# Audio-WestlakeU/NBSS

Hardware: AMD Instinct MI355X
Metric: utterances/sec (4 s, 6ch, 129 freqs) SpatialNet bf16 train at 1/2/4/8 MI355X (higher is better)
Workload: dtype bf16; 1 GPU; SpatialNet-small 6ch->2spk, 4-s 8-kHz utterances (32000 samples), n_fft 256/hop 128 (F=129, T=251), 8 layers, full train step (STFT..Adam), bf16 stream + fp32 master/stats, 32 utterances per GPU per step; batch_per_gpu=32, global_batch=32, parallelism=dp1

## Files before the change

nbss_amd/csrc/common.h:

```cpp
#pragma once
#ifdef NBSS_EMU
#include "hipemu.h"
#define NBSS_LDS(name) char* name = hipemu::g_block->lds
#else
#include <hip/hip_runtime.h>
#define NBSS_LDS(name) extern __shared__ __attribute__((aligned(16))) char name[]
#endif
#include <stdint.h>

typedef unsigned short bf16_t;
typedef float f32x4 __attribute__((ext_vector_type(4)));
typedef float f32x2 __attribute__((ext_vector_type(2)));
typedef short s16x8 __attribute__((ext_vector_type(8)));
typedef short s16x4 __attribute__((ext_vector_type(4)));
typedef unsigned int u32x2 __attribute__((ext_vector_type(2)));
typedef unsigned int u32x4 __attribute__((ext_vector_type(4)));

#define NBSS_DEV __device__ __forceinline__

NBSS_DEV float bf2f(bf16_t h) {
    union { uint32_t u; float f; } c;
    c.u = ((uint32_t)h) << 16;
    return c.f;
}
// ... 11 lines not shown
NBSS_DEV uint32_t pack2bf(float a, float b) {
    typedef __bf16 bf16x2_t __attribute__((ext_vector_type(2)));
    typedef float f32x2_t __attribute__((ext_vector_type(2)));
    f32x2_t v = {a, b};
    return __builtin_bit_cast(uint32_t, __builtin_convertvector(v, bf16x2_t));
}
#endif

NBSS_DEV float keep_if(bool c, float v) { return c ? v : 0.f; }

NBSS_DEV float fast_exp2(float x) {
#ifdef NBSS_EMU
    return exp2f(x);
#else
    return __builtin_amdgcn_exp2f(x);
#endif
}

NBSS_DEV float silu_f(float x) { return x / (1.0f + __expf(-x)); }
NBSS_DEV float dsilu_f(float x) {
    float s = 1.0f / (1.0f + __expf(-x));
    return s * (1.0f + x * (1.0f - s));
}

NBSS_DEV float fast_rcp(float x) {
#ifdef NBSS_EMU
    return 1.0f / x;
#else
    return __builtin_amdgcn_rcpf(x);
#endif
}
NBSS_DEV float sigmoid_fast(float x) { return fast_rcp(1.0f + fast_exp2(-1.44269504f * x)); }
NBSS_DEV float silu_fast(float x) { return x * sigmoid_fast(x); }
NBSS_DEV float dsilu_fast(float x) {
    const float s = sigmoid_fast(x);
    return s * (1.0f + x * (1.0f - s));
}
NBSS_DEV void silu_pair(float x, float& y, float& dy) {
    const float s = sigmoid_fast(x);
    y = x * s;
    dy = s * (1.0f + x * (1.0f - s));
}

NBSS_DEV void lds_barrier() {
#ifdef NBSS_EMU
    __syncthreads();
#else
    __builtin_amdgcn_s_waitcnt(0xC07F);
    __builtin_amdgcn_s_barrier();
#endif
}

NBSS_DEV float opaque(float x) {
#ifndef NBSS_EMU
    asm volatile("" : "+v"(x));
#endif
    return x;
}

NBSS_DEV void sched_fence() {
#ifndef NBSS_EMU
    __builtin_amdgcn_sched_barrier(0);
#endif
}

NBSS_DEV void wave_lds_sync() {
#ifdef NBSS_EMU
    hipemu::wave_sync();
#else
    __builtin_amdgcn_fence(__ATOMIC_RELEASE, "wavefront");
    __builtin_amdgcn_wave_barrier();
    __builtin_amdgcn_fence(__ATOMIC_ACQUIRE, "wavefront");
#endif
}

NBSS_DEV void dma16_to_lds(void* lds_wave_base, const void* g) {
#ifdef NBSS_EMU
    uint32_t* d = reinterpret_cast<uint32_t*>(reinterpret_cast<char*>(lds_wave_base) + 16 * (threadIdx.x & 63));
    const uint32_t* s = reinterpret_cast<const uint32_t*>(g);
    d[0] = s[0]; d[1] = s[1]; d[2] = s[2]; d[3] = s[3];
#else
    __builtin_amdgcn_global_load_lds((const __attribute__((address_space(1))) void*)g, (__attribute__((address_space(3))) void*)lds_wave_base, 16, 0, 0);
#endif
}
NBSS_DEV void dma_wait_all() {
#ifndef NBSS_EMU
    __builtin_amdgcn_s_waitcnt(0x0F70);
#endif
}

NBSS_DEV int lane_id() { return (int)(threadIdx.x & 63); }
NBSS_DEV int wave_id() { return (int)(threadIdx.x >> 6); }
NBSS_DEV int wave_id_u() {
#ifdef NBSS_EMU
    return (int)(threadIdx.x >> 6);
#else
    return __builtin_amdgcn_readfirstlane((int)(threadIdx.x >> 6));
#endif
}

NBSS_DEV float wave_sum16(float v) {
    v += __shfl_xor(v, 16);
    v += __shfl_xor(v, 32);
    return v;
}
NBSS_DEV float wave_max16(float v) {
// ... 220 lines not shown
```

nbss_amd/csrc/fconv.hip:

```cpp
#include "launch.h"
#include "layout.h"
#include "prof.h"
#include "blocks.h"
#include "wgrad.h"
#include "fold.h"
#include "foldk.h"
#include "geom.h"
#include "side.h"
#include <cstdlib>

#define FC_H 96
#define FC_G 8
#define FC_CG 12
#define FC_KS 2
#define FC_MTF_MAX 10
#define FC_MTF_BIG 17
#define FC_P16 (5 * FC_H * FC_CG)

template <class T> struct VecOf;
template <> struct VecOf<bf16_t> { static constexpr int N = 8; };
template <> struct VecOf<float> { static constexpr int N = 4; };

NBSS_DEV void vec_copy(bf16_t* d, const bf16_t* s) { *reinterpret_cast<u32x4*>(d) = *reinterpret_cast<const u32x4*>(s); }
NBSS_DEV void vec_copy(float* d, const float* s) { *reinterpret_cast<f32x4*>(d) = *reinterpret_cast<const f32x4*>(s); }
// ... 193 lines not shown

    if constexpr (REGX) {
#pragma unroll
        for (int k = 0; k < NXR; ++k) {
            const int i = tid + k * NTHR, f = i / VPR, off = (i % VPR) * VN, tt = off / HH;
            if (i >= F * VPR || t0 + tt >= T_) continue;
            const size_t go = (((size_t)b * F + f) * T_ + t0) * HH + off;
            float yv[8], o[8];
            load8(u + (size_t)f * ROW + tt * HHP + (off - tt * HH), yv);
#pragma unroll
            for (int j = 0; j < 4; ++j) {
                o[2 * j] = bf2f((bf16_t)(xr[k][j] & 0xFFFF)) + yv[2 * j];
                o[2 * j + 1] = bf2f((bf16_t)(xr[k][j] >> 16)) + yv[2 * j + 1];
            }
            store8(reinterpret_cast<bf16_t*>(y) + go, o);
        }
        for (int i = tid + NXR * NTHR; i < F * VPR; i += NTHR) {
            const int f = i / VPR, off = (i % VPR) * VN, tt = off / HH;
            if (t0 + tt >= T_) continue;
            const size_t go = (((size_t)b * F + f) * T_ + t0) * HH + off;
            float xv[8], yv[8], o[8];
            load8(x + go, xv);
            load8(u + (size_t)f * ROW + tt * HHP + (off - tt * HH), yv);
#pragma unroll
            for (int j = 0; j < 8; ++j) o[j] = xv[j] + yv[j];
            store8(reinterpret_cast<bf16_t*>(y) + go, o);
        }
    } else
    for (int i = tid; i < F * VPR; i += nthr) {
        const int f = i / VPR, off = (i % VPR) * VN, tt = off / HH;
        if (t0 + tt >= T_) continue;
        const size_t go = (((size_t)b * F + f) * T_ + t0) * HH + off;
        float xv[8], yv[8];
        if (VN == 8) {
            load8(x + go, xv);
            load8(u + (size_t)f * ROW + tt * HHP + (off - tt * HH), yv);
            float o[8];
#pragma unroll
            for (int j = 0; j < 8; ++j) o[j] = xv[j] + yv[j];
            store4(y + go, o[0], o[1], o[2], o[3]);
            store4(y + go + 4, o[4], o[5], o[6], o[7]);
        } else {
            load4(x + go, xv);
            load4(u + (size_t)f * ROW + tt * HHP + (off - tt * HH), yv);
            store4(y + go, xv[0] + yv[0], xv[1] + yv[1], xv[2] + yv[2], xv[3] + yv[3]);
        }
    }
}


#define FC_LD 104

template <class T>
NBSS_DEV void fconv_bfrag(Frag<T>& bq, const T* __restrict__ u, int rstride, int f, int ch0, int ks) {
    const int g4 = lane_id() >> 4;
    const int p0 = ks * 8 + 2 * g4, p1 = p0 + 1;
    frag_load_lo(bq, u + (size_t)(f + p0 / 3) * rstride + ch0 + (p0 % 3) * 4);
    if (p1 < 15) frag_load_hi(bq, u + (size_t)(f + p1 / 3) * rstride + ch0 + (p1 % 3) * 4);
    else frag_zero_hi(bq);
}

template <class T, bool WGF>
__global__ __launch_bounds__(64 * FC_G, 2)
void fconv_bwd_kernel(nbss_cfg c, const float* __restrict__ lnw, const float* __restrict__ lnb, const float* __restrict__ cb,
                      const float* __restrict__ slope, float* __restrict__ part, const T* __restrict__ Wp, const T* __restrict__ WpT,
                      const T* __restrict__ x, const T* __restrict__ dy, T* __restrict__ dx, float* __restrict__ stats, T* __restrict__ dvout, int flip) {
    constexpr int TT = 1, NW = FC_G;
    NBSS_LDS(smem);
    const int F = c.F, T_ = c.T, ntt = cdiv(T_, TT);
    const int bid = flip_bid(flip);
    const int b = bid / ntt, t0 = (bid % ntt) * TT;
    const int mtf = cdiv(F, 16), FP = mtf * 16 + 4, ntile = mtf * TT;
    constexpr int ROW = TT * FC_LD;
    T* u = reinterpret_cast<T*>(smem);
    T* dvb = u + (size_t)FP * ROW;
    float* aff = reinterpret_cast<float*>(dvb + (size_t)FP * ROW);
    float* lnp = aff + 3 * FC_H;
    float* affw = lnp + 2 * FC_H;
    PHASE_BEGIN(affw + NW * 2 * FC_H);
    const int tid = threadIdx.x, lane = lane_id(), l15 = lane & 15, g4 = lane >> 4, w = wave_id();
    constexpr bool DMA = sizeof(T) == 2;

    Frag<T> af[FC_KS], at[FC_KS];
#pragma unroll
    for (int ks = 0; ks < FC_KS; ++ks) {
        wfrag_load(af[ks], Wp, w < FC_G ? w : 0, FC_KS, ks);
        wfrag_load(at[ks], WpT, w < FC_G ? w : 0, FC_KS, ks);
    }
    for (int i = tid; i < 3 * FC_H; i += blockDim.x) aff[i] = 0.f;
    for (int i = tid; i < NW * 2 * FC_H; i += blockDim.x) affw[i] = 0.f;
    for (int i = tid; i < 2 * FC_H; i += blockDim.x) lnp[i] = i < FC_H ? lnw[i] : lnb[i - FC_H];
    constexpr int VZ = VecOf<T>::N;
    for (int i = tid; i < 4 * ROW / VZ; i += blockDim.x) {
        const int e = i * VZ, hr = e / ROW, rr = hr < 2 ? hr : mtf * 16 + hr, off = e % ROW;
        vec_zero(u + (size_t)rr * ROW + off);
        vec_zero(dvb + (size_t)rr * ROW + off);
    }

    auto row_load = [&](int ti, Frag<T> (&xq)[BK_KS], Frag<T> (&dq)[BK_KS]) {
        const int ft = ti / TT, tt = ti % TT, f = ft * 16 + l15, t = t0 + tt;
        const bool valid = f < F && t < T_;
        const size_t n = ((size_t)b * F + f) * T_ + t;
#pragma unroll
        for (int ks = 0; ks < BK_KS; ++ks) {
            if (valid) {
                frag_load(xq[ks], x + n * FC_H + ks * 32 + 8 * g4);
                frag_load(dq[ks], dy + n * FC_H + ks * 32 + 8 * g4);
            } else {
                frag_zero(xq[ks]);
                frag_zero(dq[ks]);
            }
        }
    };
    auto row_stats = [&](const Frag<T> (&xq)[BK_KS], float& mean, float& rstd) {
        float sum = 0.f;
#pragma unroll
        for (int ks = 0; ks < BK_KS; ++ks)
#pragma unroll
            for (int j = 0; j < 8; ++j) sum += frag_get(xq[ks], j);
        mean = wave_sum16(sum) * (1.0f / FC_H);
        float q = 0.f;
#pragma unroll
        for (int ks = 0; ks < BK_KS; ++ks)
#pragma unroll
            for (int j = 0; j < 8; ++j) {
                const float d = frag_get(xq[ks], j) - mean;
                q += d * d;
            }
        rstd = rsqrtf(wave_sum16(q) * (1.0f / FC_H) + 1e-5f);
    };
    auto row_fwd = [&](int ti, const Frag<T> (&xq)[BK_KS], const Frag<T> (&dq)[BK_KS], float mean, float rstd) {
        const int ft = ti / TT, tt = ti % TT, f = ft * 16 + l15, t = t0 + tt;
        const bool valid = f < F && t < T_;
        if (!WGF && valid && g4 == 0) {
            const size_t n = ((size_t)b * F + f) * T_ + t;
            stats[n * 2] = mean;
            stats[n * 2 + 1] = rstd;
        }
        T* ur = u + (size_t)(f + 2) * ROW + tt * FC_LD;
        T* dr_ = dvb + (size_t)(f + 2) * ROW + tt * FC_LD;
#pragma unroll
        for (int ks = 0; ks < BK_KS; ++ks) {
            const int c0 = ks * 32 + 8 * g4;
            float gm[8], bt[8], o[8], d[8];
            load8(lnp + c0, gm);
            load8(lnp + FC_H + c0, bt);
#pragma unroll
            for (int j = 0; j < 8; ++j) {
                o[j] = valid ? (frag_get(xq[ks], j) - mean) * rstd * gm[j] + bt[j] : 0.f;
                d[j] = frag_get(dq[ks], j);
            }
            store8(ur + c0, o);
            if (!DMA) store8(dr_ + c0, d);
        }
    };
    Frag<T> xr[BK_KS], dr[BK_KS];
    float rmean = 0.f, rrstd = 0.f;
    if constexpr (DMA) {
        const int wu = wave_id_u(), Q = F * TT * 13;
        for (int i = wu; i * 64 < Q; i += NW) {
            const int q = i * 64 + lane, r = q / 13, cc = q - r * 13, f = r / TT, tt = r - f * TT;
            if (q < Q && cc < 12 && t0 + tt < T_) {
                const size_t n = ((size_t)b * F + f) * T_ + t0 + tt;
                dma16_to_lds(reinterpret_cast<char*>(u + 2 * ROW) + (size_t)i * 1024, x + n * FC_H + cc * 8);
                dma16_to_lds(reinterpret_cast<char*>(dvb + 2 * ROW) + (size_t)i * 1024, dy + n * FC_H + cc * 8);
            }
        }
        for (int i = tid; i < (mtf * 16 - F) * ROW / VZ; i += blockDim.x) {
            vec_zero(u + (size_t)(F + 2) * ROW + i * VZ);
            vec_zero(dvb + (size_t)(F + 2) * ROW + i * VZ);
        }
        if (t0 + TT > T_)
            for (int i = tid; i < F * FC_LD / VZ; i += blockDim.x) {
                const int f = i / (FC_LD / VZ), e = (i % (FC_LD / VZ)) * VZ;
                for (int tt = T_ - t0; tt < TT; ++tt) {
                    vec_zero(u + (size_t)(f + 2) * ROW + tt * FC_LD + e);
                    vec_zero(dvb + (size_t)(f + 2) * ROW + tt * FC_LD + e);
                }
            }
        dma_wait_all();
        lds_barrier();
        auto row_load_lds = [&](int ti, Frag<T> (&xq)[BK_KS], Frag<T> (&dq)[BK_KS]) {
            const int ft = ti / TT, tt = ti % TT, f = ft * 16 + l15;
#pragma unroll
            for (int ks = 0; ks < BK_KS; ++ks) {
                frag_load(xq[ks], u + (size_t)(f + 2) * ROW + tt * FC_LD + ks * 32 + 8 * g4);
                frag_load(dq[ks], dvb + (size_t)(f + 2) * ROW + tt * FC_LD + ks * 32 + 8 * g4);
            }
        };
        if (w < ntile) {
            row_load_lds(w, xr, dr);
            row_stats(xr, rmean, rrstd);
            row_fwd(w, xr, dr, rmean, rrstd);
        }
        for (int ti = w + NW; ti < ntile; ti += NW) {
            Frag<T> xq[BK_KS], dq[BK_KS];
            float mean, rstd;
            row_load_lds(ti, xq, dq);
            row_stats(xq, mean, rstd);
            row_fwd(ti, xq, dq, mean, rstd);
        }
    } else {
    if (w < ntile) row_load(w, xr, dr);
    lds_barrier();
    if (w < ntile) {
        row_stats(xr, rmean, rrstd);
        row_fwd(w, xr, dr, rmean, rrstd);
    }
    for (int ti = w + NW; ti < ntile; ti += NW) {
        Frag<T> xq[BK_KS], dq[BK_KS];
        float mean, rstd;
        row_load(ti, xq, dq);
        row_stats(xq, mean, rstd);
        row_fwd(ti, xq, dq, mean, rstd);
    }
    }
    PHASE(0);
    lds_barrier();
    PHASE(1);

    const int ch = w * FC_CG + 4 * g4;
    const bool cvalid = g4 < 3;
    float cbv[4] = {0.f, 0.f, 0.f, 0.f}, slv[4] = {0.f, 0.f, 0.f, 0.f}, dsl[4] = {0.f, 0.f, 0.f, 0.f};
    if (cvalid) {
#pragma unroll
        for (int r = 0; r < 4; ++r) { cbv[r] = cb[ch + r]; slv[r] = slope[ch + r]; }
    }
    for (int ti = 0; ti < ntile; ++ti) {
        const int ft = ti / TT, tt = ti % TT, f = ft * 16 + l15;
        f32x4 acc = F32X4_ZERO;
#pragma unroll
        for (int ks = 0; ks < FC_KS; ++ks) {
            Frag<T> bq;
            fconv_bfrag<T>(bq, u + tt * FC_LD, ROW, f, w * FC_CG, ks);
            acc = mma(af[ks], bq, acc);
        }
        if (cvalid) {
            T* pd = dvb + (size_t)(f + 2) * ROW + tt * FC_LD + ch;
            float dyv[4], dv[4];
            load4(pd, dyv);
#pragma unroll
            for (int r = 0; r < 4; ++r) {
                const float v = acc[r] + cbv[r];
                dv[r] = v > 0.f ? dyv[r] : slv[r] * dyv[r];
                if (v <= 0.f) dsl[r] += dyv[r] * v;
            }
            store4(pd, dv[0], dv[1], dv[2], dv[3]);
        }
    }
#pragma unroll
    for (int r = 0; r < 4; ++r) {
        const float s2 = row_sum16(dsl[r]);
        if (l15 == 0 && cvalid) atomicAdd(aff + 2 * FC_H + ch + r, s2);
    }
    PHASE(2);
    lds_barrier();
    PHASE(3);

    constexpr int PROW = 4 * FC_H;
    if constexpr (WGF) {
        f32x4 wacc[5], bsum = F32X4_ZERO;
#pragma unroll
        for (int tap = 0; tap < 5; ++tap) wacc[tap] = F32X4_ZERO;
        Frag<T> ones;
#pragma unroll
        for (int jq = 0; jq < 8; ++jq) frag_set(ones, jq, 1.0f);
        const int nk = cdiv(mtf * 16, 32);
        const bool odd = (mtf & 1) != 0;
        const int roff = (4 * g4 + (l15 >> 2)) * ROW + w * FC_CG + 4 * (l15 & 3);
        for (int tt = 0; tt < TT; ++tt)
            for (int ks = 0; ks < nk; ++ks) {
                const bool half = odd && ks == nk - 1;
                Frag<T> fa;
                frag_load_tr(fa, dvb + (size_t)(2 + 32 * ks) * ROW + tt * FC_LD + roff, ROW);
                if (half) frag_zero_hi(fa);
                bsum = mma(fa, ones, bsum);
#pragma unroll
                for (int tap = 0; tap < 5; ++tap) {
                    Frag<T> fb;
                    frag_load_tr(fb, u + (size_t)(32 * ks + tap) * ROW + tt * FC_LD + roff, ROW);
                    if (half) frag_zero_hi(fb);
                    wacc[tap] = mma(fa, fb, wacc[tap]);
                }
            }
        bf16_t* prow16 = reinterpret_cast<bf16_t*>(part + (size_t)gridDim.x * PROW) + (size_t)bid * FC_P16;
        float* pb = part + (size_t)bid * PROW + 3 * FC_H;
        if (l15 < FC_CG && g4 < 3) {
#pragma unroll
            for (int tap = 0; tap < 5; ++tap) {
                const u32x2 v = {pack2bf(wacc[tap][0], wacc[tap][1]), pack2bf(wacc[tap][2], wacc[tap][3])};
                *reinterpret_cast<u32x2*>(prow16 + ((size_t)(tap * FC_G + w) * FC_CG + l15) * FC_CG + 4 * g4) = v;
            }
            if (l15 == 0) {
#pragma unroll
                for (int r = 0; r < 4; ++r) pb[w * FC_CG + 4 * g4 + r] = bsum[r];
            }
        }
    }

    for (int ti = 0; ti < ntile; ++ti) {
        const int ft = ti / TT, tt = ti % TT, f = ft * 16 + l15;
        f32x4 acc = F32X4_ZERO;
#pragma unroll
        for (int ks = 0; ks < FC_KS; ++ks) {
            Frag<T> bq;
            fconv_bfrag<T>(bq, dvb + tt * FC_LD, ROW, f, w * FC_CG, ks);
            acc = mma(at[ks], bq, acc);
        }
        if (cvalid) store4(u + (size_t)(f + 2) * ROW + tt * FC_LD + ch, acc[0], acc[1], acc[2], acc[3]);
    }
    if (!WGF) {
        constexpr int VN = VecOf<T>::N, VPR = FC_H / VN;
        for (int i = tid; i < F * TT * VPR; i += blockDim.x) {
            const int f = i / (TT * VPR), rem = i % (TT * VPR), tt = rem / VPR, off = (rem % VPR) * VN;
            if (t0 + tt < T_) vec_copy(dvout + (((size_t)b * F + f) * T_ + t0 + tt) * FC_H + off, dvb + (size_t)(f + 2) * ROW + tt * FC_LD + off);
        }
    }
    PHASE(4);
    lds_barrier();
    PHASE(5);

    auto row_bwd = [&](int ti, const Frag<T> (&xq)[BK_KS], const Frag<T> (&dq)[BK_KS], float mean, float rstd0) {
        const int ft = ti / TT, tt = ti % TT, f = ft * 16 + l15, t = t0 + tt;
        const bool valid = f < F && t < T_;
        const size_t n = ((size_t)b * F + f) * T_ + t;
        const T* ur = u + (size_t)(f + 2) * ROW + tt * FC_LD;
        const float rstd = valid ? rstd0 : 0.f;
        float m1 = 0.f, m2 = 0.f;
        static_assert(BK_KS == 3, "three k-steps of 32 channels");
        float* aw = affw + w * 2 * FC_H;
        float va[16];
        auto ks_vals = [&](int ks, float (&dvv)[8], float (&xhv)[8], bool stats) {
            const int c0 = ks * 32 + 8 * g4;
            float duv[8], gm[8];
            load8(ur + c0, duv);
            if (stats) load8(lnp + c0, gm);
#pragma unroll
            for (int j = 0; j < 8; ++j) {
                dvv[j] = valid ? duv[j] : 0.f;
                xhv[j] = (frag_get(xq[ks], j) - mean) * rstd;
                if (stats) {
                    m1 += dvv[j] * gm[j];
                    m2 += dvv[j] * gm[j] * xhv[j];
                }
            }
        };
        {
            float dvv[8], xhv[8];
#pragma unroll
            for (int ks = 0; ks < 2; ++ks) {
                ks_vals(ks, dvv, xhv, true);
#pragma unroll
                for (int j = 0; j < 8; ++j) va[8 * ks + j] = dvv[j] * xhv[j];
            }
            const float r0 = row_reduce16x16(va);
            aw[(l15 >> 3) * 32 + 8 * g4 + (l15 & 7)] += r0;
            ks_vals(2, dvv, xhv, true);
#pragma unroll
            for (int j = 0; j < 8; ++j) va[j] = dvv[j] * xhv[j];
#pragma unroll
            for (int j = 0; j < 8; ++j) va[8 + j] = dvv[j];
            const float r1 = row_reduce16x16(va);
            aw[(l15 >> 3) * FC_H + 64 + 8 * g4 + (l15 & 7)] += r1;
#pragma unroll
            for (int ks = 0; ks < 2; ++ks) {
                ks_vals(ks, dvv, xhv, false);
#pragma unroll
                for (int j = 0; j < 8; ++j) va[8 * ks + j] = dvv[j];
            }
            const float r2 = row_reduce16x16(va);
            aw[FC_H + (l15 >> 3) * 32 + 8 * g4 + (l15 & 7)] += r2;
        }
        m1 = wave_sum16(m1) * (1.0f / FC_H);
        m2 = wave_sum16(m2) * (1.0f / FC_H);
        if (valid) {
#pragma unroll
            for (int ks = 0; ks < BK_KS; ++ks) {
                const int c0 = ks * 32 + 8 * g4;
                float duv[8], gm[8], o[8];
                load8(ur + c0, duv);
                load8(lnp + c0, gm);
#pragma unroll
                for (int j = 0; j < 8; ++j) {
                    const float xh = (frag_get(xq[ks], j) - mean) * rstd;
                    o[j] = frag_get(dq[ks], j) + rstd * (duv[j] * gm[j] - m1 - xh * m2);
                }
                store8(dx + n * FC_H + c0, o);
            }
        }
    };
    if (w < ntile) row_bwd(w, xr, dr, rmean, rrstd);
    for (int ti = w + NW; ti < ntile; ti += NW) {
        Frag<T> xq[BK_KS], dq[BK_KS];
        float mean, rstd;
        row_load(ti, xq, dq);
        row_stats(xq, mean, rstd);
        row_bwd(ti, xq, dq, mean, rstd);
    }
    PHASE(6);
    lds_barrier();
    for (int i = threadIdx.x; i < 3 * FC_H; i += blockDim.x) {
        float v = aff[i];
        if (i < 2 * FC_H)
            for (int k = 0; k < NW; ++k) v += affw[k * 2 * FC_H + i];
        part[(size_t)bid * (WGF ? PROW : 3 * FC_H) + i] = v;
    }
    PHASE(7);
    PHASE_END();
}
PHASE_READER(nbss_phase_read_fconv_bwd)

template <class T, bool WGF>
static int fconv_bwd_t(const nbss_cfg& c, const float* P, float* part, const void* packed, int layer, int which, const void* x, const void* dy, void* dx,
                       float* stats, void* dv, hipStream_t st) {
    const int mtf = cdiv(c.F, 16);
    if (mtf > FC_MTF_BIG) return NBSS_EUNSUPPORTED;
    const size_t lds = (size_t)2 * (mtf * 16 + 4) * FC_LD * sizeof(T) + (5 + 2 * FC_G) * FC_H * sizeof(float) + PHASE_LDS_BYTES;
    if (lds > 160 * 1024) return NBSS_EUNSUPPORTED;
    const int lw = which ? P_FC2_LN_W : P_FC1_LN_W, lb = which ? P_FC2_LN_B : P_FC1_LN_B, sl = which ? P_FC2_PRELU : P_FC1_PRELU;
    const T* pk = (const T*)packed;
    int e = NBSS_SET_MAX_LDS((fconv_bwd_kernel<T, WGF>), lds);
    if (e) return e;
    dim3 grid(c.B * c.T), block(64 * FC_G);
    ProfScope ps(PK_FCONV_B, st);
    NBSS_LAUNCH((fconv_bwd_kernel<T, WGF>), grid, block, lds, st, c, P + param_off(c, layer, lw), P + param_off(c, layer, lb),
                P + param_off(c, layer, which ? P_FC2_B : P_FC1_B), P + param_off(c, layer, sl), part, pk + pack_off(c, layer, which ? K_FC2 : K_FC1),
                pk + pack_off(c, layer, which ? K_FC2_T : K_FC1_T), (const T*)x, (const T*)dy, (T*)dx, stats, (T*)dv, walk_flip_next());
    return NBSS_CHECK_LAUNCH();
}


#define TV_RSL_MAX 64
int part16_slices_launch(const void* part16, int nrows, float* slices, int p16, int* nsl, hipStream_t st, bool batch);
static_assert(FC_H == FK_H && FC_CG == FK_FCG && FC_G == FK_FG && FC_P16 == FK_FC_P16, "foldk.h");
__global__ __launch_bounds__(256) void fconv_part_final_kernel(const float* __restrict__ slices, int nsl, float* __restrict__ dW) {
    fk_fconv_final(slices, nsl, dW, (int)blockIdx.x);
}

int fconv_bwd_impl(const nbss_cfg& c, const float* P, float* G, const void* packed, int layer, int which, const void* x, const void* dy, void* dx,
                   void* ws, hipStream_t st, const Side* sd) {
    if (c.H != FC_H) return gb_fconv_bwd(c, P, G, layer, which, x, dy, dx, ws, st, sd);
    const size_t N = (size_t)c.B * c.F * c.T;
    float* stats = (float*)ws;
    void* dv = (char*)ws + ws_align(N * 2 * sizeof(float));
    float* part = (float*)((char*)ws + ws_part_offset(c));
    const bool big = c.F > 16 * FC_MTF_MAX;
    const bool fused = c.dtype == NBSS_BF16 && !big;
    if (fused) part = (float*)((char*)ws + ws_fcpart_offset(c));
    int e = c.dtype != NBSS_BF16 ? fconv_bwd_t<float, false>(c, P, part, packed, layer, which, x, dy, dx, stats, dv, st)
            : fused              ? fconv_bwd_t<bf16_t, true>(c, P, part, packed, layer, which, x, dy, dx, stats, dv, st)
                                 : fconv_bwd_t<bf16_t, false>(c, P, part, packed, layer, which, x, dy, dx, stats, dv, st);
    if (e) return e;
    const int nwg = c.B * c.T;
    AffSegs sg;
    sg.off[0] = param_off(c, layer, which ? P_FC2_LN_W : P_FC1_LN_W); sg.cnt[0] = FC_H;
    sg.off[1] = param_off(c, layer, which ? P_FC2_LN_B : P_FC1_LN_B); sg.cnt[1] = FC_H;
    sg.off[2] = param_off(c, layer, which ? P_FC2_PRELU : P_FC1_PRELU); sg.cnt[2] = FC_H;
    sg.n = fused ? 4 : 3;
    sg.off[3] = param_off(c, layer, which ? P_FC2_B : P_FC1_B); sg.cnt[3] = FC_H;
    const hipStream_t gs = side_fork(sd, st);
    FoldScope fs(gs, (char*)ws + ws_wgpart_offset(c), WGPART_BYTES, N);
    if ((e = affine_reduce_launch(part, nwg, sg, G, gs))) return e;
    if (fused) {
        float* slices = (float*)((char*)ws + ws_wgpart_offset(c));
        bool batch = false;
        if (g_fold) {
            int err;
            void* sl = g_fold->alloc((size_t)TV_RSL_MAX * FC_P16 * sizeof(float), &err);
            if (err) return err;
            if (sl) {
                slices = (float*)sl;
                batch = true;
            } else if ((err = g_fold->flush())) {
                return err;
            }
        }
        int nsl = 0;
        if ((e = part16_slices_launch(part + (size_t)nwg * 4 * FC_H, nwg, slices, FC_P16, &nsl, gs, batch))) return e;
        if (batch) {
            FoldItem it;
            it.kind = FK_FCONV_FINAL;
            it.gx = (FC_P16 + 255) / 256; it.gy = 1; it.nblk = it.gx;
            it.u.p16.part16 = nullptr; it.u.p16.nrows = nwg; it.u.p16.p16 = FC_P16; it.u.p16.nsl = nsl; it.u.p16.slices = slices;
            it.u.p16.G = G + param_off(c, layer, which ? P_FC2_W : P_FC1_W);
            if ((e = g_fold->add(2, it))) return e;
            return fs.end();
        }
        NBSS_FOLD_LAUNCH(fconv_part_final_kernel, dim3((FC_P16 + 255) / 256), dim3(256), 0, gs, (const float*)slices, nsl, G + param_off(c, layer, which ? P_FC2_W : P_FC1_W));
        return NBSS_CHECK_LAUNCH();
    }
    WgradArgs a;
    a.part = (float*)((char*)ws + ws_wgpart_offset(c));
    a.mvalid = 0; a.nvalid = 0;
    a.Ntok = (int)N; a.F = c.F; a.T = c.T; a.shift_stride = c.T; a.shift_dim = 1; a.groups = c.f_groups; a.taps = c.f_ks;
    a.A = dv; a.lda = FC_H; a.MA = FC_H; a.B = x; a.ldb = FC_H; a.NB = FC_H;
    a.stats = stats; a.gamma = P + param_off(c, layer, which ? P_FC2_LN_W : P_FC1_LN_W); a.beta = P + param_off(c, layer, which ? P_FC2_LN_B : P_FC1_LN_B);
    a.dW = G + param_off(c, layer, which ? P_FC2_W : P_FC1_W); a.dbias = G + param_off(c, layer, which ? P_FC2_B : P_FC1_B);
    if ((e = wgrad_launch(a, c.dtype, gs))) return e;
    return fs.end();
}

template <class T, int TT, int GPW, int MTF, int HH>
static int fconv_fwd_t(const nbss_cfg& c, const float* P, const void* packed, int layer, int which, const void* x, void* y, hipStream_t st) {
    const int mtf = cdiv(c.F, 16);
    if (mtf > MTF) return NBSS_EUNSUPPORTED;
    const size_t lds = (size_t)(mtf * 16 + 4) * TT * (HH + 8) * sizeof(T);
    if (lds > 160 * 1024) return NBSS_EUNSUPPORTED;
    const float* lnw = P + param_off(c, layer, which ? P_FC2_LN_W : P_FC1_LN_W);
    const float* lnb = P + param_off(c, layer, which ? P_FC2_LN_B : P_FC1_LN_B);
    const float* cb = P + param_off(c, layer, which ? P_FC2_B : P_FC1_B);
    const float* sl = P + param_off(c, layer, which ? P_FC2_PRELU : P_FC1_PRELU);
    const T* Wp = (const T*)packed + pack_off(c, layer, which ? K_FC2 : K_FC1);
    int e = NBSS_SET_MAX_LDS((fconv_fwd_kernel<T, TT, GPW, MTF, HH>), lds);
    if (e) return e;
    dim3 grid(c.B * cdiv(c.T, TT)), block(64 * FC_G / GPW);
// ... 20 lines not shown
```

nbss_amd/csrc/layout.h:

```cpp
#pragma once
#include "../../include/nbss_hip.h"

#ifdef NBSS_EMU
#define NBSS_HD inline
#else
#define NBSS_HD __host__ __device__ inline
#endif

enum LayerParam {
    P_FC1_LN_W, P_FC1_LN_B, P_FC1_W, P_FC1_B, P_FC1_PRELU,
    P_FULL_LN_W, P_FULL_LN_B, P_SQ_W, P_SQ_B, P_FULL_W, P_FULL_B, P_USQ_W, P_USQ_B,
    P_FC2_LN_W, P_FC2_LN_B, P_FC2_W, P_FC2_B, P_FC2_PRELU,
    P_MH_LN_W, P_MH_LN_B, P_INP_W, P_INP_B, P_OUTP_W, P_OUTP_B,
    P_TF_LN_W, P_TF_LN_B, P_TF_W1, P_TF_B1, P_TF_C1W, P_TF_C1B, P_TF_C2W, P_TF_C2B,
    P_TF_GN_W, P_TF_GN_B, P_TF_C3W, P_TF_C3B, P_TF_W2, P_TF_B2,
    NUM_LAYER_PARAMS
};

NBSS_HD int64_t layer_param_numel(const nbss_cfg& c, int p) {
    const int64_t H = c.H, FFN = c.FFN, SQ = c.SQ, F = c.F;
    switch (p) {
        case P_FC1_LN_W: case P_FC1_LN_B: case P_FC2_LN_W: case P_FC2_LN_B:
        case P_FULL_LN_W: case P_FULL_LN_B: case P_MH_LN_W: case P_MH_LN_B:
        case P_TF_LN_W: case P_TF_LN_B:
// ... 119 lines not shown
        case K_TF_W1_T: g.MT = c.H / 16; g.KS = c.t_groups * cdiv(cg, 32); break;
        case K_TF_C1_T: case K_TF_C2_T: case K_TF_C3_T: g.MT = cdiv(cg, 32) * 2; g.KS = cdiv(c.t_ks * (cg / 4), 8); g.NB = c.t_groups; break;
        case K_TF_W2_T: g.MT = c.t_groups * cdiv(cg, 32) * 2; g.KS = c.H / 32; break;
        case K_TF_W1_TN: g.MT = c.H / 16; g.KS = c.FFN / 32; break;
        case K_INP_TN: g.MT = c.H / 16; g.KS = 3 * c.H / 32; break;
        case K_TS_W1: g.MT = 1; g.KS = c.H / 16 + 1; g.NB = c.t_groups; break;
        case K_TS_W2_T: g.MT = 1; g.KS = c.H / 16; g.NB = c.t_groups; break;
        case K_TS_C1: case K_TS_C2: case K_TS_C3: case K_TS_C1_T: case K_TS_C2_T: case K_TS_C3_T:
            g.MT = 1; g.KS = cdiv(c.t_ks * (cg / 8) + 1, 2); g.NB = c.t_groups; break;
        case K_TS_W2: g.MT = c.H / 32; g.KS = c.FFN / 16 + 1; break;
    }
    return g;
}
NBSS_HD int ts_conv_k(int ks, int h, int j, int& tap, int& ch) {
    const int blk = 2 * ks + h;
    if (blk < 9) {
        tap = blk / 3;
        ch = (blk % 3) * 8 + j;
        return 1;
    }
    return (blk == 9 && j == 0) ? 2 : 0;
}
NBSS_HD int64_t pack_numel(const nbss_cfg& c, int kind) {
    PackGeom g = pack_geom(c, kind);
    return (int64_t)g.NB * g.MT * g.KS * 512;
}
NBSS_HD bool pack_is_global(int kind) { return kind == K_ENC || kind == K_DEC || kind == K_DEC_T; }
NBSS_HD int64_t pack_layer_numel(const nbss_cfg& c) {
    int64_t s = 0;
    for (int k = 0; k < NUM_PACK_KINDS; ++k)
        if (!pack_is_global(k)) s += pack_numel(c, k);
    return s;
}
NBSS_HD int64_t pack_off(const nbss_cfg& c, int layer, int kind) {
    if (kind == K_ENC) return 0;
    if (kind == K_DEC) return pack_numel(c, K_ENC);
    if (kind == K_DEC_T) return pack_numel(c, K_ENC) + pack_numel(c, K_DEC);
    int64_t o = pack_numel(c, K_ENC) + pack_numel(c, K_DEC) + pack_numel(c, K_DEC_T) + (int64_t)layer * pack_layer_numel(c);
    for (int k = 0; k < kind; ++k)
        if (!pack_is_global(k)) o += pack_numel(c, k);
    return o;
}
NBSS_HD int64_t pack_total(const nbss_cfg& c) {
    return pack_numel(c, K_ENC) + pack_numel(c, K_DEC) + pack_numel(c, K_DEC_T) + (int64_t)c.L * pack_layer_numel(c);
}

#define WGPART_BYTES ((size_t)512 * 112 * 272 * sizeof(float))
NBSS_HD size_t ws_align(size_t b) { return (b + 255) & ~(size_t)255; }
#define NBSS_T_TRAIN_MAX 256
#define NBSS_F_MAX 272
#define NBSS_T_MAX 4096
#define NBSS_FC_PROW(c) (4 * (c).H)
#define NBSS_FC_P16(c) ((c).H * ((c).H / (c).f_groups) * (c).f_ks)
NBSS_HD size_t fc_part_bytes(const nbss_cfg& c) { return (size_t)c.B * c.T * (NBSS_FC_PROW(c) * sizeof(float) + NBSS_FC_P16(c) * 2); }
NBSS_HD size_t tc_part_bytes(const nbss_cfg& c) {
    return c.dtype == NBSS_BF16 && c.H == 96 && c.T <= 256
               ? (size_t)c.B * c.F * ((5 * c.FFN + c.H) * sizeof(float) + ((size_t)3 * c.FFN * (c.FFN / c.t_groups) * c.t_ks + (size_t)c.FFN * c.H) * 2)
               : 0;
}
NBSS_HD size_t ws_nops(const nbss_cfg& c) { return c.H == 96 ? 8 : 16; }
NBSS_HD size_t ws_wprep_bytes(const nbss_cfg& c) { return c.H == 96 ? 0 : (size_t)16 << 20; }
NBSS_HD size_t ws_part_bytes(const nbss_cfg& c) {
    const size_t nwg = (size_t)c.B * (c.F > c.T ? c.F : c.T);
    return ws_align((nwg * 576 + 64 + (size_t)c.SQ * c.H + c.SQ + 2 * c.H) * sizeof(float));
}
NBSS_HD size_t workspace_bytes(const nbss_cfg& c) {
    const size_t N = (size_t)c.B * c.F * c.T, esz = c.dtype == NBSS_BF16 ? 2 : 4;
    return ws_align(N * 2 * sizeof(float)) + ws_nops(c) * ws_align(N * c.FFN * esz) + ws_wprep_bytes(c) + ws_part_bytes(c) + ws_align(WGPART_BYTES) +
           ws_align(fc_part_bytes(c)) + ws_align(tc_part_bytes(c)) + 256;
}
NBSS_HD size_t mhsa_lse_offset(const nbss_cfg& c) {
    return ws_align((size_t)c.B * c.F * c.T * c.H * (c.dtype == NBSS_BF16 ? 2 : 4));
}
NBSS_HD size_t mhsa_stat_offset(const nbss_cfg& c) { return mhsa_lse_offset(c) + ws_align((size_t)c.B * c.F * c.T * c.heads * sizeof(float)); }
NBSS_HD size_t mhsa_save_bytes(const nbss_cfg& c) {
    const size_t s = mhsa_stat_offset(c) + ws_align((size_t)c.B * c.F * c.T * 2 * sizeof(float));
    return (c.T > NBSS_T_TRAIN_MAX || c.H != 96) && s < 2 * mhsa_lse_offset(c) ? 2 * mhsa_lse_offset(c) : s;
}
NBSS_HD size_t ws_part_offset(const nbss_cfg& c) {
    const size_t N = (size_t)c.B * c.F * c.T, esz = c.dtype == NBSS_BF16 ? 2 : 4;
    return ws_align(N * 2 * sizeof(float)) + ws_nops(c) * ws_align(N * c.FFN * esz) + ws_wprep_bytes(c);
}

NBSS_HD size_t ws_op_offset(const nbss_cfg& c, int slot) {
    const size_t N = (size_t)c.B * c.F * c.T, esz = c.dtype == NBSS_BF16 ? 2 : 4;
    return ws_align(N * 2 * sizeof(float)) + (size_t)slot * ws_align(N * c.FFN * esz);
}
enum { WS_TC_A1 = 0, WS_TC_A2, WS_TC_A3, WS_TC_H5, WS_TC_DA1, WS_TC_Y, WS_TC_GN };

NBSS_HD size_t ws_wgpart_offset(const nbss_cfg& c) { return ws_part_offset(c) + ws_part_bytes(c); }

NBSS_HD size_t ws_fcpart_offset(const nbss_cfg& c) { return ws_wgpart_offset(c) + ws_align(WGPART_BYTES); }
NBSS_HD size_t ws_tcpart_offset(const nbss_cfg& c) { return ws_fcpart_offset(c) + ws_align(fc_part_bytes(c)); }

NBSS_HD int check_cfg(const nbss_cfg& c) {
    if (c.B <= 0 || c.F <= 0 || c.T <= 0 || c.L <= 0) return NBSS_EINVAL;
    if (c.dtype != NBSS_F32 && c.dtype != NBSS_BF16) return NBSS_EINVAL;
    const bool small = c.H == 96 && c.FFN == 192 && c.SQ == 8 && c.heads == 4;
    const bool large = c.H == 192 && c.FFN == 384 && c.SQ == 16 && c.heads == 4;
    if (!small && !large) return NBSS_EUNSUPPORTED;
    if (c.f_groups != 8 || c.t_groups != 8 || c.f_ks != 5 || c.t_ks != 3 || c.enc_ks != 5) return NBSS_EUNSUPPORTED;
    if (c.C_in % 4 != 0 || c.C_in > 16 || c.C_out > 16 || c.C_out <= 0) return NBSS_EUNSUPPORTED;
    if (c.F > NBSS_F_MAX || c.T > NBSS_T_MAX) return NBSS_EUNSUPPORTED;
    if (c.full_share < 0 || c.full_share >= c.L) return NBSS_EINVAL;
    if ((size_t)c.B * c.F * c.T * 3 * c.H >= ((size_t)1 << 31)) return NBSS_EUNSUPPORTED;
    return NBSS_OK;
}
// ... 1 lines not shown
```

Measured before the change: 735.1 utterances/s.

## Make fused bf16 frequency-conv backward a persistent kernel over frame ranges

The fused bf16 fconv backward kernel now launches about two workgroups per CU. Each workgroup walks a contiguous range of (batch, time) frames instead of handling one frame. Weight-gradient and bias accumulators stay in registers and LDS across frames and are written once per workgroup in fp32. The affine reduce can then fold the weight gradient directly, which removes the per-frame bf16 slice partials and their separate fold pass. The next frame's x/dy slabs are DMA'd into LDS while the current frame is finishing, and the weight fragments are reloaded per phase to reduce register pressure under the higher occupancy bound. The cost is less parallelism per launch and more serialized work per workgroup.

```diff
diff --git a/nbss_amd/csrc/common.h b/nbss_amd/csrc/common.h
--- a/nbss_amd/csrc/common.h
+++ b/nbss_amd/csrc/common.h
@@ -87,6 +87,13 @@
 }
 
 NBSS_DEV float opaque(float x) {
+#ifndef NBSS_EMU
+    asm volatile("" : "+v"(x));
+#endif
+    return x;
+}
+
+NBSS_DEV int opaque(int x) {
 #ifndef NBSS_EMU
     asm volatile("" : "+v"(x));
 #endif
diff --git a/nbss_amd/csrc/fconv.hip b/nbss_amd/csrc/fconv.hip
--- a/nbss_amd/csrc/fconv.hip
+++ b/nbss_amd/csrc/fconv.hip
@@ -269,24 +269,26 @@
 #define FC_LD 104
 
 template <class T>
-NBSS_DEV void fconv_bfrag(Frag<T>& bq, const T* __restrict__ u, int rstride, int f, int ch0, int ks) {
-    const int g4 = lane_id() >> 4;
+NBSS_DEV void fconv_bfrag(Frag<T>& bq, const T* __restrict__ u, int rstride, int f, int ch0, int ks, int g4) {
     const int p0 = ks * 8 + 2 * g4, p1 = p0 + 1;
     frag_load_lo(bq, u + (size_t)(f + p0 / 3) * rstride + ch0 + (p0 % 3) * 4);
     if (p1 < 15) frag_load_hi(bq, u + (size_t)(f + p1 / 3) * rstride + ch0 + (p1 % 3) * 4);
     else frag_zero_hi(bq);
 }
 
-template <class T, bool WGF>
-__global__ __launch_bounds__(64 * FC_G, 2)
+template <class T, bool WGF, bool PERS = false>
+__global__ __launch_bounds__(64 * FC_G, PERS ? 4 : 2)
 void fconv_bwd_kernel(nbss_cfg c, const float* __restrict__ lnw, const float* __restrict__ lnb, const float* __restrict__ cb,
                       const float* __restrict__ slope, float* __restrict__ part, const T* __restrict__ Wp, const T* __restrict__ WpT,
                       const T* __restrict__ x, const T* __restrict__ dy, T* __restrict__ dx, float* __restrict__ stats, T* __restrict__ dvout, int flip) {
     constexpr int TT = 1, NW = FC_G;
+    static_assert(!PERS || (WGF && sizeof(T) == 2), "the persistent walk is the fused bf16 instance's");
     NBSS_LDS(smem);
     const int F = c.F, T_ = c.T, ntt = cdiv(T_, TT);
     const int bid = flip_bid(flip);
-    const int b = bid / ntt, t0 = (bid % ntt) * TT;
+    const long long nfr = (long long)c.B * ntt;
+    const int fr0 = PERS ? (int)(bid * nfr / gridDim.x) : bid, fr1 = PERS ? (int)((bid + 1) * nfr / gridDim.x) : bid + 1;
+    int b = fr0 / ntt, t0 = (fr0 % ntt) * TT;
     const int mtf = cdiv(F, 16), FP = mtf * 16 + 4, ntile = mtf * TT;
     constexpr int ROW = TT * FC_LD;
     T* u = reinterpret_cast<T*>(smem);
@@ -294,18 +296,25 @@
     float* aff = reinterpret_cast<float*>(dvb + (size_t)FP * ROW);
     float* lnp = aff + 3 * FC_H;
     float* affw = lnp + 2 * FC_H;
-    PHASE_BEGIN(affw + NW * 2 * FC_H);
-    const int tid = threadIdx.x, lane = lane_id(), l15 = lane & 15, g4 = lane >> 4, w = wave_id();
+    float* affb = affw + NW * 2 * FC_H;
+    PHASE_BEGIN(affb + FC_H);
+    int tid = threadIdx.x, lane = lane_id(), l15 = lane & 15, g4 = lane >> 4, w = wave_id();
     constexpr bool DMA = sizeof(T) == 2;
 
     Frag<T> af[FC_KS], at[FC_KS];
-#pragma unroll
-    for (int ks = 0; ks < FC_KS; ++ks) {
-        wfrag_load(af[ks], Wp, w < FC_G ? w : 0, FC_KS, ks);
-        wfrag_load(at[ks], WpT, w < FC_G ? w : 0, FC_KS, ks);
+    auto wfrags = [&](Frag<T> (&a)[FC_KS], const T* __restrict__ wp) {
+#pragma unroll
+        for (int ks = 0; ks < FC_KS; ++ks) {
+            if constexpr (PERS) frag_load(a[ks], wp + ((size_t)(w * FC_KS + ks) * 64 + lane) * 8);
+            else wfrag_load(a[ks], wp, w < FC_G ? w : 0, FC_KS, ks);
+        }
+    };
+    if constexpr (!PERS) {
+        wfrags(af, Wp);
+        wfrags(at, WpT);
     }
     for (int i = tid; i < 3 * FC_H; i += blockDim.x) aff[i] = 0.f;
-    for (int i = tid; i < NW * 2 * FC_H; i += blockDim.x) affw[i] = 0.f;
+    for (int i = tid; i < (NW * 2 + 1) * FC_H; i += blockDim.x) affw[i] = 0.f;
     for (int i = tid; i < 2 * FC_H; i += blockDim.x) lnp[i] = i < FC_H ? lnw[i] : lnb[i - FC_H];
     constexpr int VZ = VecOf<T>::N;
     for (int i = tid; i < 4 * ROW / VZ; i += blockDim.x) {
@@ -322,7 +331,7 @@
         for (int ks = 0; ks < BK_KS; ++ks) {
             if (valid) {
                 frag_load(xq[ks], x + n * FC_H + ks * 32 + 8 * g4);
-                frag_load(dq[ks], dy + n * FC_H + ks * 32 + 8 * g4);
+                if constexpr (!PERS) frag_load(dq[ks], dy + n * FC_H + ks * 32 + 8 * g4);
             } else {
                 frag_zero(xq[ks]);
                 frag_zero(dq[ks]);
@@ -371,17 +380,55 @@
             if (!DMA) store8(dr_ + c0, d);
         }
     };
+    f32x4 wacc[5];
+#pragma unroll
+    for (int tap = 0; tap < 5; ++tap) wacc[tap] = F32X4_ZERO;
+    constexpr int PROW = PERS ? 4 * FC_H + FC_P16 : 4 * FC_H;
+    auto wgrad_row_store = [&](const f32x4 (&wa)[5], const f32x4& bs) {
+        bf16_t* prow16 = reinterpret_cast<bf16_t*>(part + (size_t)gridDim.x * PROW) + (size_t)bid * FC_P16;
+        float* pb = part + (size_t)bid * PROW + 3 * FC_H;
+        if constexpr (PERS) {
+            float* pw = part + (size_t)bid * PROW + 4 * FC_H;
+            if (l15 < FC_CG && g4 < 3) {
+#pragma unroll
+                for (int tap = 0; tap < 5; ++tap)
+#pragma unroll
+                    for (int r = 0; r < 4; ++r) pw[((size_t)(w * FC_CG + 4 * g4 + r) * FC_CG + l15) * 5 + tap] = wa[tap][r];
+            }
+        } else if (l15 < FC_CG && g4 < 3) {
+#pragma unroll
+            for (int tap = 0; tap < 5; ++tap) {
+                const u32x2 v = {pack2bf(wa[tap][0], wa[tap][1]), pack2bf(wa[tap][2], wa[tap][3])};
+                *reinterpret_cast<u32x2*>(prow16 + ((size_t)(tap * FC_G + w) * FC_CG + l15) * FC_CG + 4 * g4) = v;
+            }
+            if (l15 == 0) {
+#pragma unroll
+                for (int r = 0; r < 4; ++r) pb[w * FC_CG + 4 * g4 + r] = bs[r];
+            }
+        }
+    };
+    auto slab_dma = [&](T* img, const T* __restrict__ src, int bb, int tb) {
+        const int wu = wave_id_u(), Q = F * TT * 13;
+        for (int i = wu; i * 64 < Q; i += NW) {
+            const int q = i * 64 + lane, r = q / 13, cc = q - r * 13, f = r / TT, tt = r - f * TT;
+            if (q < Q && cc < 12 && tb + tt < T_) {
+                const size_t n = ((size_t)bb * F + f) * T_ + tb + tt;
+                dma16_to_lds(reinterpret_cast<char*>(img + 2 * ROW) + (size_t)i * 1024, src + n * FC_H + cc * 8);
+            }
+        }
+    };
+    for (int fr = fr0; fr < fr1; ++fr) {
+    b = fr / ntt, t0 = (fr % ntt) * TT;
+    if constexpr (PERS) {
+        tid = opaque(tid);
+        lane = tid & 63, l15 = lane & 15, g4 = lane >> 4, w = tid >> 6;
+    }
     Frag<T> xr[BK_KS], dr[BK_KS];
     float rmean = 0.f, rrstd = 0.f;
     if constexpr (DMA) {
-        const int wu = wave_id_u(), Q = F * TT * 13;
-        for (int i = wu; i * 64 < Q; i += NW) {
-            const int q = i * 64 + lane, r = q / 13, cc = q - r * 13, f = r / TT, tt = r - f * TT;
-            if (q < Q && cc < 12 && t0 + tt < T_) {
-                const size_t n = ((size_t)b * F + f) * T_ + t0 + tt;
-                dma16_to_lds(reinterpret_cast<char*>(u + 2 * ROW) + (size_t)i * 1024, x + n * FC_H + cc * 8);
-                dma16_to_lds(reinterpret_cast<char*>(dvb + 2 * ROW) + (size_t)i * 1024, dy + n * FC_H + cc * 8);
-            }
+        if (!PERS || fr == fr0) {
+            slab_dma(u, x, b, t0);
+            slab_dma(dvb, dy, b, t0);
         }
         for (int i = tid; i < (mtf * 16 - F) * ROW / VZ; i += blockDim.x) {
             vec_zero(u + (size_t)(F + 2) * ROW + i * VZ);
@@ -405,12 +452,12 @@
                 frag_load(dq[ks], dvb + (size_t)(f + 2) * ROW + tt * FC_LD + ks * 32 + 8 * g4);
             }
         };
-        if (w < ntile) {
+        if (!PERS && w < ntile) {
             row_load_lds(w, xr, dr);
             row_stats(xr, rmean, rrstd);
             row_fwd(w, xr, dr, rmean, rrstd);
         }
-        for (int ti = w + NW; ti < ntile; ti += NW) {
+        for (int ti = PERS ? w : w + NW; ti < ntile; ti += NW) {
             Frag<T> xq[BK_KS], dq[BK_KS];
             float mean, rstd;
             row_load_lds(ti, xq, dq);
@@ -439,6 +486,7 @@
     const int ch = w * FC_CG + 4 * g4;
     const bool cvalid = g4 < 3;
     float cbv[4] = {0.f, 0.f, 0.f, 0.f}, slv[4] = {0.f, 0.f, 0.f, 0.f}, dsl[4] = {0.f, 0.f, 0.f, 0.f};
+    if constexpr (PERS) wfrags(af, Wp);
     if (cvalid) {
 #pragma unroll
         for (int r = 0; r < 4; ++r) { cbv[r] = cb[ch + r]; slv[r] = slope[ch + r]; }
@@ -449,7 +497,7 @@
 #pragma unroll
         for (int ks = 0; ks < FC_KS; ++ks) {
             Frag<T> bq;
-            fconv_bfrag<T>(bq, u + tt * FC_LD, ROW, f, w * FC_CG, ks);
+            fconv_bfrag<T>(bq, u + tt * FC_LD, ROW, f, w * FC_CG, ks, g4);
             acc = mma(af[ks], bq, acc);
         }
         if (cvalid) {
@@ -471,14 +519,12 @@
         if (l15 == 0 && cvalid) atomicAdd(aff + 2 * FC_H + ch + r, s2);
     }
     PHASE(2);
+    if constexpr (PERS) wfrags(at, WpT);
     lds_barrier();
     PHASE(3);
 
-    constexpr int PROW = 4 * FC_H;
     if constexpr (WGF) {
-        f32x4 wacc[5], bsum = F32X4_ZERO;
-#pragma unroll
-        for (int tap = 0; tap < 5; ++tap) wacc[tap] = F32X4_ZERO;
+        f32x4 bsum = F32X4_ZERO;
         Frag<T> ones;
 #pragma unroll
         for (int jq = 0; jq < 8; ++jq) frag_set(ones, jq, 1.0f);
@@ -500,18 +546,10 @@
                     wacc[tap] = mma(fa, fb, wacc[tap]);
                 }
             }
-        bf16_t* prow16 = reinterpret_cast<bf16_t*>(part + (size_t)gridDim.x * PROW) + (size_t)bid * FC_P16;
-        float* pb = part + (size_t)bid * PROW + 3 * FC_H;
-        if (l15 < FC_CG && g4 < 3) {
-#pragma unroll
-            for (int tap = 0; tap < 5; ++tap) {
-                const u32x2 v = {pack2bf(wacc[tap][0], wacc[tap][1]), pack2bf(wacc[tap][2], wacc[tap][3])};
-                *reinterpret_cast<u32x2*>(prow16 + ((size_t)(tap * FC_G + w) * FC_CG + l15) * FC_CG + 4 * g4) = v;
-            }
-            if (l15 == 0) {
-#pragma unroll
-                for (int r = 0; r < 4; ++r) pb[w * FC_CG + 4 * g4 + r] = bsum[r];
-            }
+        if constexpr (!PERS) wgrad_row_store(wacc, bsum);
+        else if (l15 == 0 && g4 < 3) {
+#pragma unroll
+            for (int r = 0; r < 4; ++r) affb[w * FC_CG + 4 * g4 + r] += bsum[r];
         }
     }
 
@@ -521,7 +559,7 @@
 #pragma unroll
         for (int ks = 0; ks < FC_KS; ++ks) {
             Frag<T> bq;
-            fconv_bfrag<T>(bq, dvb + tt * FC_LD, ROW, f, w * FC_CG, ks);
+            fconv_bfrag<T>(bq, dvb + tt * FC_LD, ROW, f, w * FC_CG, ks, g4);
             acc = mma(at[ks], bq, acc);
         }
         if (cvalid) store4(u + (size_t)(f + 2) * ROW + tt * FC_LD + ch, acc[0], acc[1], acc[2], acc[3]);
@@ -536,6 +574,9 @@
     PHASE(4);
     lds_barrier();
     PHASE(5);
+    const int bn = (fr + 1) / ntt, tn = ((fr + 1) % ntt) * TT;
+    if constexpr (PERS)
+        if (fr + 1 < fr1) slab_dma(dvb, dy, bn, tn);
 
     auto row_bwd = [&](int ti, const Frag<T> (&xq)[BK_KS], const Frag<T> (&dq)[BK_KS], float mean, float rstd0) {
         const int ft = ti / TT, tt = ti % TT, f = ft * 16 + l15, t = t0 + tt;
@@ -595,19 +636,21 @@
             for (int ks = 0; ks < BK_KS; ++ks) {
                 const int c0 = ks * 32 + 8 * g4;
                 float duv[8], gm[8], o[8];
+                Frag<T> dl;
+                if constexpr (PERS) frag_load(dl, dy + n * FC_H + c0);
                 load8(ur + c0, duv);
                 load8(lnp + c0, gm);
 #pragma unroll
                 for (int j = 0; j < 8; ++j) {
                     const float xh = (frag_get(xq[ks], j) - mean) * rstd;
-                    o[j] = frag_get(dq[ks], j) + rstd * (duv[j] * gm[j] - m1 - xh * m2);
+                    o[j] = frag_get(PERS ? dl : dq[ks], j) + rstd * (duv[j] * gm[j] - m1 - xh * m2);
                 }
                 store8(dx + n * FC_H + c0, o);
             }
         }
     };
-    if (w < ntile) row_bwd(w, xr, dr, rmean, rrstd);
-    for (int ti = w + NW; ti < ntile; ti += NW) {
+    if (!PERS && w < ntile) row_bwd(w, xr, dr, rmean, rrstd);
+    for (int ti = PERS ? w : w + NW; ti < ntile; ti += NW) {
         Frag<T> xq[BK_KS], dq[BK_KS];
         float mean, rstd;
         row_load(ti, xq, dq);
@@ -616,7 +659,14 @@
     }
     PHASE(6);
     lds_barrier();
-    for (int i = threadIdx.x; i < 3 * FC_H; i += blockDim.x) {
+    if constexpr (PERS)
+        if (fr + 1 < fr1) slab_dma(u, x, bn, tn);
+    }
+    if constexpr (PERS) {
+        wgrad_row_store(wacc, F32X4_ZERO);
+        for (int i = tid; i < FC_H; i += blockDim.x) part[(size_t)bid * PROW + 3 * FC_H + i] = affb[i];
+    }
+    for (int i = tid; i < 3 * FC_H; i += blockDim.x) {
         float v = aff[i];
         if (i < 2 * FC_H)
             for (int k = 0; k < NW; ++k) v += affw[k * 2 * FC_H + i];
@@ -627,20 +677,35 @@
 }
 PHASE_READER(nbss_phase_read_fconv_bwd)
 
-template <class T, bool WGF>
+static int fconv_bwd_pers_grid(int nframes) {
+#ifdef NBSS_EMU
+    const int ncu = 4;
+#else
+    static const int ncu = [] {
+        int dev = 0, n = 0;
+        if (hipGetDevice(&dev) != hipSuccess || hipDeviceGetAttribute(&n, hipDeviceAttributeMultiprocessorCount, dev) != hipSuccess || n <= 0) n = 256;
+        return n;
+    }();
+#endif
+    const int g = 2 * ncu < NBSS_FC_PERS_ROWS_MAX ? 2 * ncu : NBSS_FC_PERS_ROWS_MAX;
+    return nframes < g ? nframes : g;
+}
+
+template <class T, bool WGF, bool PERS = false>
 static int fconv_bwd_t(const nbss_cfg& c, const float* P, float* part, const void* packed, int layer, int which, const void* x, const void* dy, void* dx,
-                       float* stats, void* dv, hipStream_t st) {
+                       float* stats, void* dv, hipStream_t st, int* nrows) {
     const int mtf = cdiv(c.F, 16);
     if (mtf > FC_MTF_BIG) return NBSS_EUNSUPPORTED;
-    const size_t lds = (size_t)2 * (mtf * 16 + 4) * FC_LD * sizeof(T) + (5 + 2 * FC_G) * FC_H * sizeof(float) + PHASE_LDS_BYTES;
+    const size_t lds = (size_t)2 * (mtf * 16 + 4) * FC_LD * sizeof(T) + (6 + 2 * FC_G) * FC_H * sizeof(float) + PHASE_LDS_BYTES;
     if (lds > 160 * 1024) return NBSS_EUNSUPPORTED;
     const int lw = which ? P_FC2_LN_W : P_FC1_LN_W, lb = which ? P_FC2_LN_B : P_FC1_LN_B, sl = which ? P_FC2_PRELU : P_FC1_PRELU;
     const T* pk = (const T*)packed;
-    int e = NBSS_SET_MAX_LDS((fconv_bwd_kernel<T, WGF>), lds);
+    int e = NBSS_SET_MAX_LDS((fconv_bwd_kernel<T, WGF, PERS>), lds);
     if (e) return e;
-    dim3 grid(c.B * c.T), block(64 * FC_G);
+    *nrows = PERS ? fconv_bwd_pers_grid(c.B * c.T) : c.B * c.T;
+    dim3 grid(*nrows), block(64 * FC_G);
     ProfScope ps(PK_FCONV_B, st);
-    NBSS_LAUNCH((fconv_bwd_kernel<T, WGF>), grid, block, lds, st, c, P + param_off(c, layer, lw), P + param_off(c, layer, lb),
+    NBSS_LAUNCH((fconv_bwd_kernel<T, WGF, PERS>), grid, block, lds, st, c, P + param_off(c, layer, lw), P + param_off(c, layer, lb),
                 P + param_off(c, layer, which ? P_FC2_B : P_FC1_B), P + param_off(c, layer, sl), part, pk + pack_off(c, layer, which ? K_FC2 : K_FC1),
                 pk + pack_off(c, layer, which ? K_FC2_T : K_FC1_T), (const T*)x, (const T*)dy, (T*)dx, stats, (T*)dv, walk_flip_next());
     return NBSS_CHECK_LAUNCH();
@@ -664,20 +729,27 @@
     const bool big = c.F > 16 * FC_MTF_MAX;
     const bool fused = c.dtype == NBSS_BF16 && !big;
     if (fused) part = (float*)((char*)ws + ws_fcpart_offset(c));
-    int e = c.dtype != NBSS_BF16 ? fconv_bwd_t<float, false>(c, P, part, packed, layer, which, x, dy, dx, stats, dv, st)
-            : fused              ? fconv_bwd_t<bf16_t, true>(c, P, part, packed, layer, which, x, dy, dx, stats, dv, st)
-                                 : fconv_bwd_t<bf16_t, false>(c, P, part, packed, layer, which, x, dy, dx, stats, dv, st);
+#ifdef NBSS_FCONV_BWD_PER_FRAME
+    constexpr bool pers = false;
+#else
+    constexpr bool pers = true;
+#endif
+    int nwg = 0;
+    int e = c.dtype != NBSS_BF16 ? fconv_bwd_t<float, false>(c, P, part, packed, layer, which, x, dy, dx, stats, dv, st, &nwg)
+            : fused              ? fconv_bwd_t<bf16_t, true, pers>(c, P, part, packed, layer, which, x, dy, dx, stats, dv, st, &nwg)
+                                 : fconv_bwd_t<bf16_t, false>(c, P, part, packed, layer, which, x, dy, dx, stats, dv, st, &nwg);
     if (e) return e;
-    const int nwg = c.B * c.T;
     AffSegs sg;
     sg.off[0] = param_off(c, layer, which ? P_FC2_LN_W : P_FC1_LN_W); sg.cnt[0] = FC_H;
     sg.off[1] = param_off(c, layer, which ? P_FC2_LN_B : P_FC1_LN_B); sg.cnt[1] = FC_H;
     sg.off[2] = param_off(c, layer, which ? P_FC2_PRELU : P_FC1_PRELU); sg.cnt[2] = FC_H;
-    sg.n = fused ? 4 : 3;
+    sg.n = fused ? (pers ? 5 : 4) : 3;
     sg.off[3] = param_off(c, layer, which ? P_FC2_B : P_FC1_B); sg.cnt[3] = FC_H;
+    sg.off[4] = param_off(c, layer, which ? P_FC2_W : P_FC1_W); sg.cnt[4] = FC_P16;
     const hipStream_t gs = side_fork(sd, st);
     FoldScope fs(gs, (char*)ws + ws_wgpart_offset(c), WGPART_BYTES, N);
     if ((e = affine_reduce_launch(part, nwg, sg, G, gs))) return e;
+    if (fused && pers) return fs.end();
     if (fused) {
         float* slices = (float*)((char*)ws + ws_wgpart_offset(c));
         bool batch = false;
diff --git a/nbss_amd/csrc/layout.h b/nbss_amd/csrc/layout.h
--- a/nbss_amd/csrc/layout.h
+++ b/nbss_amd/csrc/layout.h
@@ -195,7 +195,13 @@
 #define NBSS_T_MAX 4096
 #define NBSS_FC_PROW(c) (4 * (c).H)
 #define NBSS_FC_P16(c) ((c).H * ((c).H / (c).f_groups) * (c).f_ks)
-NBSS_HD size_t fc_part_bytes(const nbss_cfg& c) { return (size_t)c.B * c.T * (NBSS_FC_PROW(c) * sizeof(float) + NBSS_FC_P16(c) * 2); }
+#define NBSS_FC_PERS_ROWS_MAX 1024
+#define NBSS_FC_PROW_PERS(c) (NBSS_FC_PROW(c) + NBSS_FC_P16(c))
+NBSS_HD size_t fc_part_bytes(const nbss_cfg& c) {
+    const size_t nfr = (size_t)c.B * c.T, per_frame = nfr * (NBSS_FC_PROW(c) * sizeof(float) + NBSS_FC_P16(c) * 2);
+    const size_t pers = (nfr < NBSS_FC_PERS_ROWS_MAX ? nfr : (size_t)NBSS_FC_PERS_ROWS_MAX) * NBSS_FC_PROW_PERS(c) * sizeof(float);
+    return per_frame > pers ? per_frame : pers;
+}
 NBSS_HD size_t tc_part_bytes(const nbss_cfg& c) {
     return c.dtype == NBSS_BF16 && c.H == 96 && c.T <= 256
                ? (size_t)c.B * c.F * ((5 * c.FFN + c.H) * sizeof(float) + ((size_t)3 * c.FFN * (c.FFN / c.t_groups) * c.t_ks + (size_t)c.FFN * c.H) * 2)
```

Result: no change. 733.3 utterances/s (-0.2%).
